# MurpheyLab/trep

Measured on AMD Instinct MI355X. Metric: DEL-steps/sec x batch (puppet ~40-DOF, fp64), higher is better.
Workload: dtype f64

## Files before the change

trep_amd/csrc/mvi_core.hpp:

```cpp
#pragma once
#include <cmath>

#include "program.hpp"
#include "dual.hpp"
#include "lanes.hpp"

#if defined(TG_MOCK_TIMING) || defined(TG_MOCK_REAL_LDS) || defined(TG_MOCK_LDS_D1) || defined(TG_MOCK_LDS_D2) || \
    defined(TG_BBD_FUSED_UPDATE) || defined(TG_BBD_INLINE) || defined(TG_BBD_ASM) || \
    defined(TG_WEV_NO_RC_IDENT) || defined(TG_WEV_CLEAR_EARLY) || defined(TG_WEV_MERGE_C) || \
    defined(TG_NO_BBD) || defined(TG_NO_CMP) || defined(TG_NO_GJ_PANEL) || defined(TG_NO_QUAD_SWEEP) || defined(TG_NO_DUAL_SWEEP) || \
    defined(TG_NO_AB_MFMA) || defined(TG_NO_HZ_MFMA) || defined(GJR_EXEC32) || defined(GJP_SKIP_STEPS) || defined(GJP_SKIP_UPDATE) || \
    defined(TG_FRESH_PHASES) || defined(TG_FRESH_STEP) || \
    defined(TG_CHAIN_PRIO) || defined(TG_PREFIX_GROUP) || defined(TG_LT_TRIPS) || defined(TG_ROLLOUT_WAVES) || defined(TG_DERIV_WAVES)
#error "a retired experiment switch is defined (TG_MOCK_*, TG_BBD_FUSED_UPDATE / _INLINE / _ASM, TG_WEV_*, TG_NO_* except TG_NO_WEV, GJR_ / GJP_*, TG_FRESH_*, or a former -D tunable): these variants were removed -- verdicts in docs/LOG.md, their source in commit 89f6ce0"
#endif

#if defined(TG_HELPER_WAVES)
constexpr int TG_NW = TG_HELPER_WAVES;
#else
constexpr int TG_NW = 1;
#endif

#if defined(__HIPCC__)
__device__ __forceinline__ double *tg_lds_base() {
// ... 48 lines not shown
template <class P> struct tg_is_spec<P, typename std::enable_if<(P::nq >= 0)>::type> { static constexpr bool value = true; };
template <class P, class = void> struct tg_items_aligned { static constexpr bool value = false; };
template <class P> struct tg_items_aligned<P, typename std::enable_if<(P::nq >= 0)>::type> { static constexpr bool value = (P::o_J % 2 == 0) && (P::o_W % 2 == 0); };
template <class P, class = void> struct tg_static_sweep { static constexpr bool value = false; };
template <class P> struct tg_static_sweep<P, typename std::enable_if<(P::sw_ok > 0)>::type> { static constexpr bool value = true; };
template <class P, class = void> struct tg_static_cmp { static constexpr bool value = false; };
template <class P> struct tg_static_cmp<P, typename std::enable_if<(P::cmp_ok >= 0)>::type> { static constexpr bool value = P::cmp_ok != 0 && P::tab_ok != 0; };

template <class P, class = void> struct tg_static_wev { static constexpr bool value = false; };
#if !defined(TG_NO_WEV)
template <class P> struct tg_static_wev<P, typename std::enable_if<(P::wev_ok >= 0)>::type> { static constexpr bool value = P::wev_ok != 0 && P::cmp_ok != 0 && P::tab_ok != 0; };
#endif

template <class P, class = void> struct tg_static_pk { static constexpr bool value = false; };
#if defined(TG_BBD_PACKED)
template <class P> struct tg_static_pk<P, typename std::enable_if<(P::bbd_pk_ok >= 0)>::type> { static constexpr bool value = P::bbd_pk_ok != 0 && tg_static_wev<P>::value && tg_static_bbd<P>::value; };
#endif

template <class P, class = void> struct tg_static_fb { static constexpr bool value = false; };
template <class P> struct tg_static_fb<P, typename std::enable_if<(P::fb_on >= 0)>::type> { static constexpr bool value = P::fb_on != 0 && tg_static_wev<P>::value; };

template <class P, class = void> struct tg_static_tr { static constexpr bool value = false; };
template <class P> struct tg_static_tr<P, typename std::enable_if<(P::tr_on >= 0)>::type> { static constexpr bool value = P::tr_on != 0 && tg_static_sweep<P>::value && P::tab_ok != 0; };

enum { MODE_ROLLOUT = 0, MODE_CALC_P2 = 1, MODE_CALC_F = 2, MODE_DERIV1 = 3, MODE_DERIV2Z = 4, MODE_DYNAMICS = 5, MODE_DYN_DERIV1 = 6, MODE_ENERGY = 7, MODE_LAGRANGIAN = 8 };

struct RunArgs {
    int batch, n_steps, max_iterations, mode;
    int predictor;
    double dt, t1, t2, tolerance;
    double *q1, *q2, *p1, *p2, *lam, *u1;
    const double *U, *K;
    const double *q2_hint, *lam_hint;
    const double *Kproj, *bX, *bU;
    double *Uout;
    int group_size;
    const int *group_map;
    double *X;
    double *f_out;
    double *d1[12];
    double *A_out, *B_out;
    const double *z;
    double *hz;
    int *iters, *status;
    long long *prof_out;
    const double *dt_steps;
// ... 352 lines not shown
                TG_SYNC();
            }
            return;
        }
#endif
        for (int L = 1; L < P.n_levels; L++) {
            const int l0 = P.level_off[L], cnt = P.level_off[L + 1] - l0;
            if (on) TG_FOR(idx, 4 * cnt) {
                const int j = P.lvl_joints[l0 + (idx >> 2)], cc = idx & 3;
                if (P.j_parent[j] < 0) continue;
                const Real *gp = G + 12 * P.j_parent[j];
                Real *gj = G + 12 * j;
                const Real m0 = gj[cc], m1 = gj[4 + cc], m2 = gj[8 + cc], u3 = (cc == 3) ? 1.0 : 0.0;
                const Real v0 = gp[0] * m0 + gp[1] * m1 + gp[2] * m2 + u3 * gp[3];
                const Real v1 = gp[4] * m0 + gp[5] * m1 + gp[6] * m2 + u3 * gp[7];
                const Real v2 = gp[8] * m0 + gp[9] * m1 + gp[10] * m2 + u3 * gp[11];
                gj[cc] = v0; gj[4 + cc] = v1; gj[8 + cc] = v2;
            }
            TG_SYNC();
        }
    }

#if defined(__HIP_DEVICE_COMPILE__)
    TG_HD void pose_sweep_dual(bool on, bool rollout_lists) {
        const int sjn = rollout_lists ? P.n_sj : 2 * P.n_joints;
        double *sc = S + P.o_sc, *sc2 = S + P.o_J, *G = S + P.o_G, *G2 = S + P.o_W;
        const int nj = P.n_joints;
        const int n12 = 12 * nj, n24 = 2 * n12;
        SwDesc sw0;
        if constexpr (tg_static_sweep<typename std::remove_cv<PROG>::type>::value) {
            if (rollout_lists) sw0 = sw_fetch<typename std::remove_cv<PROG>::type, 0>((const int *)(S + SwPlan<typename std::remove_cv<PROG>::type>::o_sched()));
        }
        constexpr bool TR = tg_static_tr<typename std::remove_cv<PROG>::type>::value;
        if (P.tab_ok) {
            double pr[2][12];
            int trw[2] = {0, 0};
#pragma unroll
            for (int u = 0; u < 2; u++) {
                const double *src = (TR && rollout_lists ? P.tr_prm : P.j_prm) + 12 * (size_t)((jck[u] >> 16) & 0xFFF);
#pragma unroll
                for (int e = 0; e < 12; e++) pr[u][e] = src[e];
                if constexpr (TR) { if (rollout_lists) trw[u] = P.tr_sj[lane + u * TEAM < sjn ? lane + u * TEAM : 0]; }
            }
            if (on) {
#pragma unroll
                for (int u = 0; u < 2; u++) {
                    const int idx = lane + u * TEAM;
                    if (u * TEAM < sjn && idx < sjn) {
                        const bool second = (jck[u] >> 28) != 0;
                        const int j = (jck[u] >> 16) & 0xFFF, kind = (jck[u] >> 12) & 0xF;
                        const double x = qval(second ? dsB : dsA, jck[u] & 0xFFF);
                        const bool rotary = kind >= TG_RX;
                        const int a = rotary ? kind - TG_RX : kind - TG_TX, b = a == 2 ? 0 : a + 1, c = a == 0 ? 2 : a - 1;
                        double *g = (second ? G2 : G) + 12 * j;
                        auto row_t = [&](int l, double v) {
                            if constexpr (TR) {
                                typedef typename std::remove_cv<PROG>::type SP;
                                constexpr int ROWS = tg_static_wev<SP>::value ? SP::tr_rows : 7;
                                if (rollout_lists && ((ROWS >> l) & 1)) { const double e = qval(second ? dsB : dsA, (trw[u] >> (8 * l)) & 0xFF); return (trw[u] >> (24 + l)) & 1 ? e : v; }
                            }
                            return v;
                        };
                        if (u * TEAM < sc_rot2) {
                            double sn = 0.0, cs = 1.0;
                            if (rotary) tg_sincos(x, &sn, &cs);
                            const double tq = rotary ? 0.0 : x;
#pragma unroll
                            for (int l = 0; l < 3; l++) {
                                const double A_ = pr[u][4 * l], B_ = pr[u][4 * l + 1], C_ = pr[u][4 * l + 2], D_ = pr[u][4 * l + 3];
                                g[4 * l + a] = A_;
                                g[4 * l + b] = rotary ? fma(C_, sn, B_ * cs) : B_;
// ... 520 lines not shown
        v += tg_dpp_f64<0x111>(v); v += tg_dpp_f64<0x112>(v); v += tg_dpp_f64<0x114>(v); v += tg_dpp_f64<0x118>(v);
        double norm2 = tg_readlane_f64(v, 15);
        if (P.nd > 16) norm2 += tg_readlane_f64(v, 31);
        if (P.nd > 32) norm2 += tg_readlane_f64(v, 47);
        if (P.nd > 48) norm2 += tg_readlane_f64(v, 63);
        return !(norm2 > tolerance * tolerance) && !__any(res_hoff ? 1 : 0);
    }

    template <int D0, int D1> TG_HD void wev_sum(const double *SU, double (&V)[6]) const {
        if constexpr (D0 < D1) {
            double x[D1 - D0][6];
#pragma unroll
            for (int d = D0; d < D1; d++) {
                const int idx = (wvl[d >> 2] >> (8 * (d & 3))) & 0xFF;
                ld6<true>(SU + 6 * idx, x[d - D0]);
            }
#pragma unroll
            for (int d = D0; d < D1; d++) {
#pragma unroll
                for (int r = 0; r < 6; r++) V[r] += x[d - D0][r];
            }
        }
    }
    TG_HD void eval_world(bool on) {
        typedef typename std::remove_cv<PROG>::type SP;
        constexpr bool FB = tg_static_fb<SP>::value;
        constexpr int nd = SP::nd, NB = SP::n_bodies, NG = SP::n_cgroups, MAXD = FB ? SP::fb_depth : SP::wev_depth;
        static_assert(TEAM == 64 && nd + 3 * NB < 64, "eval_world: one lane per config and per (body, axis), and the last lane free");
        static_assert(!FB || nd + 3 * NB < 63, "eval_world: the prefix record needs a second lane without a role");
        constexpr int NREC = (SP::o_ccz - SP::o_csw) / 12;
        static_assert((SP::o_ccz - SP::o_csw) % 12 == 0 && NREC == nd + (FB ? 2 : 1), "eval_world: the twist area holds nd + 1 records, nd + 2 with a prefix");
        static_assert((SP::o_csw & 1) == 0 && ((SP::o_csw + 6 * NREC) & 1) == 0 && (SP::o_I & 1) == 0 && (SP::o_cmp & 1) == 0 && (SP::o_G & 1) == 0, "eval_world: 16-byte LDS accesses");
        const int l0 = tg_opaque(lane);
        const bool blane = l0 >= nd && l0 < nd + 3 * NB;
        const int wb_ = blane ? wvl[3] & 0xFF : 0, wr_ = blane ? (wvl[3] >> 8) & 3 : 0;
        double eo0, eo1, eo2, eor; int eanc;
        {
            const int ii = l0 < 3 * P.n_endpoints ? l0 : 0;
            const double *o = P.ae_d + 4 * (size_t)ii;
            eo0 = o[0]; eo1 = o[1]; eo2 = o[2]; eor = o[3]; eanc = P.ae_i[ii];
        }
        double Cb[12];
#pragma unroll
        for (int e = 0; e < 12; e++) Cb[e] = P.b_C[12 * (size_t)wb_ + e];
        const int banc = P.b_anchor[wb_];
        if (!rates_ready) {
            if (on) TG_FOR(i, P.nq) S[P.o_dq + i] = (S[P.o_q2 + i] - S[P.o_q1 + i]) / dt;
            TG_RSYNC();
        }
        TG_STAMP(0);
        pose_sweep_dual(on, true);
        TG_STAMP(1);
        const double *G = S + P.o_G, *G2 = S + P.o_W;
        double *SW = S + P.o_csw, *SU = SW + 6 * NREC, *CMP = S + P.o_cmp, *BW = S + P.o_W + 12 * P.n_joints;
        constexpr int BWS = 17;
        static_assert(12 * SP::n_joints + BWS * NB <= 6 * SP::n_items + 9 * NB, "eval_world: body entries do not fit behind the q2 poses");
        const ConTab ct = fetch_constraints();
        double bD0 = 0.0, bD1 = 0.0, bD2 = 0.0, bC0 = 0.0, bC1 = 0.0, bC2 = 0.0, bm = 0.0;
        if (on) {
            if (lane < 3 * P.n_endpoints) {
                const int r = lane % 3;
                const double *g = G2 + 12 * (eanc < 0 ? 0 : eanc) + 4 * r;
                const double val = g[0] * eo0 + g[1] * eo1 + g[2] * eo2 + g[3];
                S[P.o_pE + lane] = eanc < 0 ? eor : val;
            }
            if (lane < nd || lane == TEAM - 1 || (FB && lane == TEAM - 2)) {
                const bool real = lane < nd;
                const int rec = real ? lane : (FB && lane == TEAM - 2 ? nd + 1 : nd);
                const int oj = real ? wvl[3] & 0xFFFF : 0, kind = real ? (wvl[3] >> 16) & 0xFF : (int)TG_TX;
                const bool prismatic = kind <= TG_TZ;
                const int ax = prismatic ? kind - TG_TX : kind - TG_RX;
                const double *gj = G + oj;
                const double a0 = gj[ax], a1 = gj[4 + ax], a2 = gj[8 + ax];
                const double px = gj[3], py = gj[7], pz = gj[11];
// ... 2760 lines not shown
        if (live && lane == 0) { A.iters[t] = 0; A.status[t] = ok ? TG_OK : TG_SINGULAR; }
    }
    if constexpr (MODE == MODE_DYNAMICS) {
        const bool ok = core.dynamics(live, A, t);
        if (live && lane == 0) { A.iters[t] = 0; A.status[t] = ok ? TG_OK : TG_SINGULAR; }
    }
}

template <int TEAM, int MODE, bool SPRINGS = false, class PROG = CProg, class ARGS = CArgs, int PIVOT = -1, bool PAR = false>
TG_HD void run_trajectory(PROG &P0, ARGS &A0, double *S, int lane, int traj, int wave = 0, int nw = 1, const ParTable T = ParTable{nullptr, 1, 0}) {
    PROG &P = P0;
    ARGS &A = A0;
    const int nq = P.nq, nd = P.nd, nk = P.nk, nu = P.nu, nc = P.nc;
    const bool live = traj < A.batch;
    const size_t t = (size_t)(live ? traj : 0);
    double dt = MODE == MODE_ROLLOUT ? A.dt : (A.t2 - A.t1);
    if (A.dt_steps && A.dt_period > 0) dt = A.dt_steps[t % (size_t)A.dt_period];
    Core<TEAM, SPRINGS, PROG, double, PAR> core(P, S, lane, dt);
    if constexpr (PAR) core.par = T.rows + (t / (size_t)T.group) * (size_t)T.stride + 4 * P.n_bodies;
    else (void)T;
    core.wave = wave; core.nw = nw;
    core.d1_compact = MODE == MODE_DERIV1 && P.a_ok != 0;
    if (wave == 0) core.init_sweep_schedule(MODE == MODE_ROLLOUT);
#if defined(TG_PROFILE) && defined(__HIP_DEVICE_COMPILE__)
    core.prof_last = (long long)__builtin_amdgcn_s_memtime();
    const long long prof_rt0 = (long long)__builtin_amdgcn_s_memrealtime();
#endif

    if (live && wave == 0) {
        TG_FOR(i, nq) { S[P.o_q1 + i] = A.q1[t * nq + i]; S[P.o_q2 + i] = A.q2[t * nq + i]; }
        TG_FOR(i, nd) S[P.o_p1 + i] = (MODE == MODE_ROLLOUT) ? A.p2[t * nd + i] : A.p1[t * nd + i];
        TG_FOR(i, nc) S[P.o_lam + i] = A.lam[t * nc + i];
        TG_FOR(i, nu) S[P.o_u + i] = A.u1[t * nu + i];
        TG_FOR(i, P.n_dh) { S[P.o_Dh1 + i] = 0.0; S[P.o_Dh2 + i] = 0.0; }
    }
    TG_SYNC();

    if constexpr (MODE == MODE_CALC_P2) {
        core.eval_midpoint(live);
        if (live) TG_FOR(i, nd) A.p2[t * nd + i] = 0.5 * dt * S[P.o_Ldq + i] + S[P.o_Lddq + i];
        return;
    }
    if constexpr (MODE == MODE_DERIV1) {
        core.deriv1(live, A, t);
        return;
    }
// ... 158 lines not shown
        if (!edged) {
        if (fuse_rates && on) TG_FOR(i, nq) S[P.o_dq + i] = core.over_dt(S[P.o_q2 + i] - S[P.o_q1 + i]);
        if (step == 0) core.eval_constraints(on, 1, false, S + P.o_Dh1);
        else if (nc) {
            if (on) TG_FOR(i, P.n_dh) S[P.o_Dh1 + i] = S[P.o_Dh2 + i];
            TG_RSYNC();
        }
        }
        int iterations = 0;
        bool done = !on;
        pre_ok = false;
        if (TEAM == 64 && on && !A.Kproj && nu <= TEAM && nk <= TEAM && step + 1 < A.n_steps) {
            if (lane < nu) pre_u = A.U[(t * A.n_steps + step + 1) * nu + lane];
            if (pre_kl >= 0 && pre_kl < nk) pre_k = A.K[(t * A.n_steps + step + 1) * nk + pre_kl];
            pre_ok = true;
        }
#if defined(TG_PROFILE) && defined(__HIP_DEVICE_COMPILE__)
        { long long t_ = (long long)__builtin_amdgcn_s_memtime(); core.prof[9] += t_ - core.prof_last; core.prof_last = t_; }
#endif
        for (;;) {
            PROG &P = tg_rebind(P0);
            const int nd = P.nd, nc = P.nc;
#if defined(__HIP_DEVICE_COMPILE__)
            if constexpr (TEAM == 64 && !SPRINGS && tg_static_wev<typename std::remove_cv<PROG>::type>::value) { core.wev_on = true; core.pk_image = PIVOT == 0; core.eval_world(!done); }
            else if (core.dual_ok()) { if (P.tab_ok) core.eval_both_tab(!done); else core.eval_both(!done); }
            else
#endif
            {
                core.eval_midpoint(!done);
                core.eval_constraints(!done, 2, true, S + P.o_Dh2);
            }
#if defined(__HIP_DEVICE_COMPILE__)
            if (core.dual_ok() && P.tab_ok) { if (!done && core.solved_fused(A.tolerance)) done = true; }
            else
#endif
            if (!done && core.solved(A.tolerance)) done = true;
#if defined(TG_PROFILE) && defined(__HIP_DEVICE_COMPILE__)
            { long long t_ = (long long)__builtin_amdgcn_s_memtime(); core.prof[12] += t_ - core.prof_last; core.prof_last = t_; }
#endif
            if (!done && iterations > A.max_iterations) { done = true; failed = true; status = TG_NOT_CONVERGED; }
#if defined(__HIP_DEVICE_COMPILE__)
            if (TEAM == 64 ? done : (__all(done ? 1 : 0) != 0)) break;
#else
            if (done) break;
#endif
#if defined(__HIP_DEVICE_COMPILE__)
            BbdRows<tg_static_bbd_cols<TEAM == 64 && PIVOT == 0, typename std::remove_cv<PROG>::type>::value> bbd_tab_rows;
// ... 172 lines not shown
```

trep_amd/csrc/program.hpp:

```cpp
#pragma once
#include "../../include/trep_amd.h"

namespace tg {

struct DevProg {
#define TG_F_INT(name) int name;
#define TG_F_ARRAY(type, name, n) type name[n];
#define TG_F_TABLE(type, name) const type *name;
#include "devprog_fields.def"
#undef TG_F_INT
#undef TG_F_ARRAY
#undef TG_F_TABLE
};

constexpr int kCmpRecord = 16, kCmpStride = 18;
static_assert(kCmpStride >= kCmpRecord && kCmpStride % 2 == 0 && kCmpRecord % 2 == 0, "composite records: 16-byte aligned");
template <class SP> constexpr int cmp_stride() {
    static_assert(SP::n_cgroups > 0 && (SP::o_csw - SP::o_cmp) % SP::n_cgroups == 0, "composite records: o_csw is not a whole number of strides behind o_cmp");
    constexpr int stride = (SP::o_csw - SP::o_cmp) / SP::n_cgroups;
    static_assert((stride == kCmpRecord || stride == kCmpStride) && (SP::o_cmp & 1) == 0, "composite records: stride");
    return stride;
}

}

#ifndef __HIPCC__
#include "schedule.hpp"
#endif
```

trep_amd/csrc/schedule.hpp:

```cpp
#pragma once
#include <algorithm>
#include <cmath>
#include <cstdio>
#include <cstdlib>
#include <cstring>
#include <functional>
#include <map>
#include <stdexcept>
#include <string>
#include <vector>

#include "program.hpp"
#include "bbd.hpp"

namespace tg {

struct HostProgram {
    DevProg p{};
#define TG_F_INT(name)
#define TG_F_ARRAY(type, name, n)
#define TG_F_TABLE(type, name) std::vector<type> name;
#include "devprog_fields.def"
#undef TG_F_INT
#undef TG_F_ARRAY
#undef TG_F_TABLE
    std::vector<unsigned char> newton_pattern;
    int max_depth = 0;
    std::vector<int> frame_anchor;
    std::vector<double> frame_offset;
    std::vector<int> ipool;
    std::vector<double> dpool;
    std::vector<size_t> toff;
    void pack();
    void bind(DevProg &P, const int *I, const double *D) const;
};

namespace detail {
struct M34 {
    double m[12];
};
inline M34 ident() {
    M34 r{};
    r.m[0] = r.m[5] = r.m[10] = 1.0;
    return r;
}
inline M34 mul(const M34 &a, const M34 &b) {
    M34 r{};
    for (int i = 0; i < 3; i++)
        for (int j = 0; j < 4; j++) {
            double s = (j == 3) ? a.m[4 * i + 3] : 0.0;
            for (int k = 0; k < 3; k++) s += a.m[4 * i + k] * b.m[4 * k + j];
            r.m[4 * i + j] = s;
// ... 28 lines not shown
    DevProg &P;
    const int nfr, nq, nd, nc;
    int n_levels = 0, nj = 0, nb = 0, nitems = 0;
    int n_true_springs = 0, ns = 0, nw = 0, nel = 0;
    int n_dh_con = 0, n_dh_spr = 0, n_cpair_con = 0, n_cpair_spr = 0;
    bool has_plane = false;
    std::vector<int> jorder, joint_of_frame, joint_of_cfg;
    std::vector<int> anchor;
    std::vector<M34> offset;
    std::map<int, int> ep_of_frame;
    int cmp_stride = kCmpRecord;
    std::vector<int> pose_need;
    int off = 0;
    static constexpr int kCompositeMinNd = 8;
    int take(int n) { int o = off; off += (n > 0 ? n : 0); return o; }

    explicit ScheduleBuilder(const tg_system_desc *desc) : d(desc), P(H.p), nfr(desc->n_frames), nq(desc->n_configs), nd(desc->n_dyn), nc(desc->n_constraints) {}
    int endpoint(int f);
    void check_desc(), number_joints(), joint_tables(), bodies_and_items();
    void constraints(), springs_and_point_forces(), element_tables(), forces_and_potentials();
    void counts_and_step_layout(), sweep_lists_and_plan(), layout_pose_union_and_deriv1();
    void body_chunks(), helper_wave_lists(), layout_derivatives();
    void composite_form(), floating_base_tables(const std::vector<std::vector<int>> &lists), world_eval();
    void structured_solve(), translation_runs();
};

inline int ScheduleBuilder::endpoint(int f) {
    auto it = ep_of_frame.find(f);
    if (it != ep_of_frame.end()) return it->second;
    int e = (int)H.e_anchor.size();
    ep_of_frame[f] = e;
    H.e_anchor.push_back(anchor[f]);
    H.e_off.push_back(offset[f].m[3]); H.e_off.push_back(offset[f].m[7]); H.e_off.push_back(offset[f].m[11]);
    return e;
}

inline void ScheduleBuilder::check_desc() {
    if (nd + d->n_kin != nq) throw std::runtime_error("n_dyn + n_kin != n_configs");
    for (int f = 0; f < nfr; f++) {
        int t = d->frame_transform[f];
        if (t < TG_WORLD || t > TG_CONST_SE3) throw std::runtime_error("unknown frame transform");
        if (d->frame_config[f] >= 0 && (t < TG_TX || t > TG_RZ)) throw std::runtime_error("config on a non-parametric frame");
        if (f > 0 && (d->frame_parent[f] < 0 || d->frame_parent[f] >= f)) throw std::runtime_error("frames must be listed parent-first");
    }
}

inline void ScheduleBuilder::number_joints() {
// ... 806 lines not shown
            const int first = H.ch_first[c] + k, len = H.ch_len[c] - k, parent = k ? first - 1 : H.ch_parent[c];
            if (len == 0) continue;
            w[0] = (12 * first) | (len << 16); w[1] = parent >= 0 ? 12 * parent : -1;
            for (int set = 0; set < 2; set++) if (pose_need[first] >> set & 1) inst.push_back(slot | (set << 8) | (1 << 9));
        }
        P.tr_np[r] = ((int)inst.size() + 4) / 5;
        for (int p = 0; p < P.tr_np[r]; p++) {
            int len = 0;
            for (int q = 0; q < 5 && 5 * p + q < (int)inst.size(); q++) {
                P.tr_inst[(4 * r + p) * 5 + q] = inst[5 * p + q];
                len = std::max(len, H.tr_sched[2 * (size_t)(16 * r + (inst[5 * p + q] & 0xFF))] >> 16);
            }
            P.tr_len[4 * r + p] = len;
            P.tr_maxlen = std::max(P.tr_maxlen, len);
        }
    }
    if (on) {
        P.tr_on = 1;
        P.o_sched2 = P.lds_per_team;
        P.lds_per_team += 16 * P.n_rounds;
    }
    if (H.tr_joint.empty()) { H.tr_joint.push_back(0); H.tr_src.assign(3, -1); H.tr_const.assign(3, 0.0); }
}
}

inline HostProgram build_program(const tg_system_desc *d) {
    detail::ScheduleBuilder b(d);
    b.check_desc(); b.number_joints(); b.joint_tables(); b.bodies_and_items();
    b.constraints(); b.springs_and_point_forces(); b.element_tables(); b.forces_and_potentials();
    b.counts_and_step_layout(); b.sweep_lists_and_plan(); b.layout_pose_union_and_deriv1();
    b.body_chunks(); b.helper_wave_lists(); b.layout_derivatives();
    b.composite_form(); b.world_eval(); b.structured_solve(); b.translation_runs();
    b.H.pack();
    return std::move(b.H);
}

namespace detail {
template <typename T>
inline size_t pool_append(std::vector<T> &pool, const std::vector<T> &v) {
    const size_t at = pool.size();
    pool.insert(pool.end(), v.begin(), v.end());
    while (pool.size() % 4) pool.push_back(T());
    return at;
}
inline std::vector<int> &pool_of(std::vector<int> &I, std::vector<double> &, int) { return I; }
inline std::vector<double> &pool_of(std::vector<int> &, std::vector<double> &D, double) { return D; }
inline const int *pool_of(const int *I, const double *, int) { return I; }
inline const double *pool_of(const int *, const double *D, double) { return D; }
inline std::string spec_value(int v) { return std::to_string(v); }
inline std::string spec_value(double v) { char t[40]; std::snprintf(t, sizeof(t), "%a", v); return t; }
template <typename T>
inline void emit_spec_pool(std::string &out, const char *decl, const std::vector<T> &pool, size_t per_line) {
    out += decl + std::to_string(pool.size()) + "] = {";
    for (size_t i = 0; i < pool.size(); i++) out += (i ? ((i % per_line) ? "," : ",\n") : "\n") + spec_value(pool[i]);
    out += "};\n";
// ... 44 lines not shown
    DevProg P = H.p;
    H.bind(P, H.ipool.data(), H.dpool.data());
    out += "// specialised schedule: sizes, counts, LDS offsets and tables as compile-time constants\n";
    detail::emit_spec_pool(out, "__device__ const int spec_ipool[", H.ipool, 32);
    detail::emit_spec_pool(out, "__device__ const double spec_dpool[", H.dpool, 8);
    out += "struct SpecProg {\n";
#define TG_F_INT(name) out += "    static constexpr int " #name " = " + std::to_string(P.name) + ";\n";
#define TG_F_ARRAY(type, name, n)
#define TG_F_TABLE(type, name)
#include "devprog_fields.def"
#undef TG_F_INT
#undef TG_F_ARRAY
#define TG_F_INT(name)
#define TG_F_ARRAY(type, name, n) detail::emit_spec_array(out, #type, #name, P.name, n);
#include "devprog_fields.def"
#undef TG_F_ARRAY
#undef TG_F_TABLE
#define TG_F_ARRAY(type, name, n)
#define TG_F_TABLE(type, name) detail::emit_spec_pointer(out, #type, #name, P.name, H);
#include "devprog_fields.def"
#undef TG_F_INT
#undef TG_F_ARRAY
#undef TG_F_TABLE
    out += "};\n";
}

}
```

trep_amd/csrc/spec_kernel.hip:

```cpp
#include <hip/hip_runtime.h>

#include <type_traits>

#define TG_GJ_PANEL_DEFAULT 1
#include "mvi_core.hpp"
#include TG_SPEC_HEADER

namespace {
#if defined(SPEC_ARGS_IN_MEMORY)
#define SPEC_KERNEL_ARGS const tg::RunArgs *__restrict__ Ag
#define SPEC_ARGS_REF tg::KArgs &A = *(tg::KArgs *)Ag
#else
#define SPEC_KERNEL_ARGS const tg::RunArgs A
#define SPEC_ARGS_REF ((void)0)
#endif

template <int MODE> constexpr int spec_waves() { return ((MODE == tg::MODE_DERIV1 || MODE == tg::MODE_DERIV2Z) && SPEC_TEAM == 64) ? TG_NW : 1; }
static_assert(TG_NW >= 1 && TG_NW <= 2, "helper waves: the pair lists of program.hpp are split in exactly two parts (wave_part, wp_* / wt_* / wcp4)");
static_assert(TG_NW == 1 || SPEC_TEAM == 64, "helper waves are for full-wave teams (trep_amd/specialize.py passes TG_HELPER_WAVES only then)");

constexpr int TG_ROLLOUT_WAVES = 2;
constexpr int TG_DERIV_WAVES = 1;
template <int MODE, int PIVOT = 0>
__global__ __launch_bounds__(64 * spec_waves<MODE>(), MODE == tg::MODE_DERIV1 ? (SpecProg::a_ok ? 2 : 1) : (MODE == tg::MODE_DERIV2Z ? TG_DERIV_WAVES : TG_ROLLOUT_WAVES)) void k_spec(SPEC_KERNEL_ARGS) {
// ... 95 lines not shown
#else
    hipLaunchKernelGGL((k_spec_par<MODE, PIVOT>), dim3(grid), dim3(64 * spec_waves<MODE>()), lds, stream, *A, T);
#endif
    return hipGetLastError() == hipSuccess ? 0 : 1;
}
}

extern "C" {
const int *tg_spec_sizes(void) {
    static const int s[8] = {(int)sizeof(tg::DevProg), (int)sizeof(tg::RunArgs), SpecProg::nq, SpecProg::nd, SpecProg::nc, SpecProg::n_items,
                             SpecProg::n_pairs, SpecProg::lds_per_team};
    return s;
}
unsigned long long tg_spec_key(void) {
#if defined(TG_SPEC_KEY)
    return TG_SPEC_KEY;
#else
    return 0ull;
#endif
}
int tg_spec_waves(void) { return spec_waves<tg::MODE_DERIV2Z>(); }
int tg_spec_fb_n(void) { return tg::tg_static_fb<SpecProg>::value ? SpecProg::fb_n : 0; }
int tg_spec_tr_n(void) { return tg::tg_static_tr<SpecProg>::value ? SpecProg::tr_n : 0; }
int tg_spec_modes(void) {
    int m = 1 << tg::MODE_ROLLOUT;
#if defined(SPEC_DERIVATIVES)
    m |= (1 << tg::MODE_DERIV1) | (1 << tg::MODE_DERIV2Z);
#endif
    return m;
}
int tg_spec_par_modes(void) { return tg_spec_modes(); }
int tg_spec_debug_solve(const double *A_dev, double *x_dev, int *path_dev, int n_mats, int skip_structured) {
    const size_t lds = sizeof(double) * (size_t)SpecProg::lds_per_team;
    if (lds > 64 * 1024 &&
        hipFuncSetAttribute(reinterpret_cast<const void *>(&k_spec_debug_solve), hipFuncAttributeMaxDynamicSharedMemorySize, (int)lds) != hipSuccess) return 1;
    hipLaunchKernelGGL(k_spec_debug_solve, dim3(n_mats), dim3(64), lds, 0, A_dev, x_dev, path_dev, skip_structured);
    return hipGetLastError() == hipSuccess ? 0 : 1;
}
int tg_spec_launch(int mode, const tg::RunArgs *A, tg::RunArgs *device_slot, int grid, size_t lds, void *stream) {
    switch (mode) {
    case tg::MODE_ROLLOUT:
        return A->exact_pivot ? launch_mode<tg::MODE_ROLLOUT, 1>(A, device_slot, grid, lds, (hipStream_t)stream)
                              : launch_mode<tg::MODE_ROLLOUT, 0>(A, device_slot, grid, lds, (hipStream_t)stream);
#if defined(SPEC_DERIVATIVES)
    case tg::MODE_DERIV1: return launch_mode<tg::MODE_DERIV1>(A, device_slot, grid, lds, (hipStream_t)stream);
    case tg::MODE_DERIV2Z: return launch_mode<tg::MODE_DERIV2Z>(A, device_slot, grid, lds, (hipStream_t)stream);
// ... 19 lines not shown
```

trep_amd/csrc/trepamd.hip:

```cpp
#include <hip/hip_runtime.h>

#include <cmath>
#include <cstdio>
#include <cstdlib>
#include <cstring>
#include <memory>
#include <string>
#include <vector>

#include "device_buffer.hpp"
#include "launch_generic.hpp"
#include "mvi_project.hpp"
#include "mvi_equilibrium.hpp"
#include "mvi_inverse.hpp"
#include "mvi_frames.hpp"
#include "mvi_tape.hpp"
#include "mvi_dyn_inverse.hpp"
#include "schedule.hpp"
#include <dlfcn.h>

namespace tg_detail {
int launch_par(int team, bool springs, const tg::DevProg *d_prog, const tg::RunArgs &A, const tg::ParTable &T, int grid, size_t lds, hipStream_t stream);
int launch_project(int team, bool springs, const tg::DevProg *d_prog, const tg::RunArgs &A, const tg::ProjectArgs &J, int grid, size_t lds, hipStream_t stream);
int launch_equilibrium(int team, bool springs, bool par, const tg::DevProg *d_prog, const tg::RunArgs &A, const tg::EquilibriumArgs &J, const tg::ParTable &T, int grid, size_t lds, hipStream_t stream);
// ... 50 lines not shown

struct tg_batch {
    tg_system *sys = nullptr;
    int batch = 0, device = 0;
    tg::DevProg P{};
    tg::DeviceBuffer<tg::DevProg> d_prog;
    void *spec_lib = nullptr;
    int (*spec_launch)(int, const tg::RunArgs *, tg::RunArgs *, int, size_t, void *) = nullptr;
    int (*spec_launch_par)(int, const tg::RunArgs *, tg::RunArgs *, int, size_t, void *, const double *, int, int) = nullptr;
    int spec_par_modes = 0;
    tg::DeviceBuffer<double> par_dev;
    int par_rows = 0, par_group = 1, par_stride = 0;
    struct Launched { unsigned int modes = 0; long long n = 0; void add(int mode) { modes |= 1u << mode; n++; } } launched[2][2];
    static constexpr int ARG_SLOTS = 4;
    tg::DeviceBuffer<tg::RunArgs> d_args;
    tg::PinnedBuffer<tg::RunArgs> h_args;
    tg::Event arg_done[ARG_SLOTS];
    bool arg_used[ARG_SLOTS] = {false, false, false, false};
    int arg_next = 0;
    tg::PinnedBuffer<double> io_host;
    double *io_dev = nullptr;
    size_t io_in = 0, io_out = 0;
    bool mirror_valid = false;
    int spec_modes = 0, spec_waves = 1, spec_fb_n = 0, spec_tr_n = 0;
    std::string spec_path;
    tg::DeviceBuffer<int> d_ints;
    tg::DeviceBuffer<double> d_dbls;
    tg::DeviceBuffer<double> q1, q2, p1, p2, lam, u1;
    tg::DeviceBuffer<double> stage_u, stage_k, stage_qh, stage_lh, f_out;
    tg::DeviceBuffer<int> iters, status, fallbacks;
    tg::DeviceBuffer<double> z_dev, hz_dev, zl_dev;
    tg::DeviceBuffer<double> dyn;
    tg::DeviceBuffer<double> dyn_d1;
    tg::DeviceBuffer<double> energy;
    tg::DeviceBuffer<double> lag;
    tg::DeviceBuffer<int> dyn_ints;
    tg::DeviceBuffer<double> pose;
    tg::DeviceBuffer<int> pose_ints;
    std::vector<int32_t> frames_sel;
    std::vector<int> frames_tab_host;
    std::vector<double> frames_off_host;
    tg::DeviceBuffer<int> frames_tab;
    tg::DeviceBuffer<double> frames_off;
    std::vector<int32_t> tape_start, tape_sel;
    tg::TapeTable tape_host;
    tg::DeviceBuffer<int> tape_words;
    tg::DeviceBuffer<double> tape_off;
// ... 1815 lines not shown
    const tg::DevProg &P = b->P;
    const int want[8] = {(int)sizeof(tg::DevProg), (int)sizeof(tg::RunArgs), P.nq, P.nd, P.nc, P.n_items, P.n_pairs, P.lds_per_team};
    const int *got = sizes_fn();
    for (int i = 0; i < 8; i++) if (got[i] != want[i]) return fail(TG_ERR_INVALID, "specialised kernel was built for a different system or library version");
    if (key_fn() != tg_system_spec_key(b->sys)) return fail(TG_ERR_INVALID, "specialised kernel was built from a different schedule (header hash mismatch)");
    if (!b->d_args) {
        tg::DeviceBuffer<tg::RunArgs> d_args;
        tg::PinnedBuffer<tg::RunArgs> h_args;
        tg::Event done[tg_batch::ARG_SLOTS];
        bool ok = d_args.ensure(tg_batch::ARG_SLOTS) == hipSuccess && h_args.ensure(tg_batch::ARG_SLOTS, hipHostMallocDefault) == hipSuccess;
        for (int i = 0; i < tg_batch::ARG_SLOTS && ok; i++) ok = done[i].create(hipEventDisableTiming) == hipSuccess;
        if (!ok) return fail(TG_ERR_HIP, "allocation of the argument blocks failed");
        b->d_args = std::move(d_args); b->h_args = std::move(h_args);
        for (int i = 0; i < tg_batch::ARG_SLOTS; i++) b->arg_done[i] = std::move(done[i]);
    }
    if (b->spec_lib) { hipStreamSynchronize(b->stream); dlclose(b->spec_lib); }
    b->spec_lib = lib.release(); b->spec_launch = launch_fn; b->spec_modes = modes_fn(); b->spec_path = library_path;
    auto waves_fn = reinterpret_cast<int (*)(void)>(dlsym(h, "tg_spec_waves"));
    b->spec_waves = waves_fn ? waves_fn() : 1;
    auto fb_fn = reinterpret_cast<int (*)(void)>(dlsym(h, "tg_spec_fb_n"));
    b->spec_fb_n = fb_fn ? fb_fn() : 0;
    auto tr_fn = reinterpret_cast<int (*)(void)>(dlsym(h, "tg_spec_tr_n"));
    b->spec_tr_n = tr_fn ? tr_fn() : 0;
    auto par_fn = reinterpret_cast<int (*)(int, const tg::RunArgs *, tg::RunArgs *, int, size_t, void *, const double *, int, int)>(dlsym(h, "tg_spec_launch_par"));
    auto par_modes_fn = reinterpret_cast<int (*)(void)>(dlsym(h, "tg_spec_par_modes"));
    b->spec_launch_par = par_modes_fn ? par_fn : nullptr;
    b->spec_par_modes = (par_fn && par_modes_fn) ? par_modes_fn() : 0;
    return TG_SUCCESS;
}

int tg_system_newton_plan(const tg_system *sys, int32_t out[8], uint8_t *pattern, int32_t *tab) {
    if (!sys || !out) return fail(TG_ERR_INVALID, "null argument");
    const tg::DevProg &P = sys->H.p;
    out[0] = P.bbd_ok; out[1] = P.bbd_g; out[2] = P.bbd_ng; out[3] = P.bbd_nb; out[4] = P.bbd_t; out[5] = P.nf; out[6] = P.nd; out[7] = 0;
    if (pattern) {
        std::memset(pattern, 0, (size_t)P.nf * P.nf);
        if (sys->H.newton_pattern.size() == (size_t)P.nf * P.nf) std::memcpy(pattern, sys->H.newton_pattern.data(), sys->H.newton_pattern.size());
    }
    if (tab) for (int i = 0; i < 128; i++) tab[i] = i < (int)sys->H.bbd_tab.size() ? sys->H.bbd_tab[i] : 0;
    return TG_SUCCESS;
}

int tg_batch_debug_newton_solve(tg_batch *b, int32_t n_mats, int32_t skip_structured, const double *A_aug_host, double *x_host, int32_t *path_host) {
    if (!b || n_mats <= 0 || !A_aug_host || !x_host || !path_host) return fail(TG_ERR_INVALID, "bad arguments");
    if (!b->spec_lib) return fail(TG_ERR_INVALID, "no specialised kernel library loaded");
    auto fn = reinterpret_cast<int (*)(const double *, double *, int *, int, int)>(dlsym(b->spec_lib, "tg_spec_debug_solve"));
    if (!fn) return fail(TG_ERR_INVALID, "the specialised library has no solve hook");
    const int nf = b->P.nf;
    HIP_TRY(hipSetDevice(b->device));
    tg::DeviceBuffer<double> dA, dx;
    tg::DeviceBuffer<int> dp;
    const size_t cA = (size_t)n_mats * nf * (nf + 1), cx = (size_t)n_mats * nf, cp = (size_t)n_mats;
    auto failed = [](const char *what) { (void)hipGetLastError(); return fail(TG_ERR_HIP, what); };
    if (dA.ensure(cA) != hipSuccess || dx.ensure(cx) != hipSuccess || dp.ensure(cp) != hipSuccess) return failed("solve hook: device allocation failed");
    if (hipMemcpy(dA.get(), A_aug_host, cA * sizeof(double), hipMemcpyHostToDevice) != hipSuccess) return failed("solve hook: upload failed");
    const int rc = fn(dA.get(), dx.get(), dp.get(), n_mats, skip_structured);
    if (hipDeviceSynchronize() != hipSuccess || rc != 0) return failed("solve hook launch failed");
    if (hipMemcpy(x_host, dx.get(), cx * sizeof(double), hipMemcpyDeviceToHost) != hipSuccess ||
        hipMemcpy(path_host, dp.get(), cp * sizeof(int), hipMemcpyDeviceToHost) != hipSuccess)
        return failed("solve hook: download failed");
    return TG_SUCCESS;
}

int tg_batch_info(const tg_batch *b, int32_t out[8]) {
    if (!b || !out) return fail(TG_ERR_INVALID, "null argument");
    out[0] = b->spec_launch ? b->spec_modes : 0;
    for (int spec = 0; spec < 2; spec++) { out[2 - spec] = (int32_t)b->launched[0][spec].modes; out[4 - spec] = (int32_t)std::min<long long>(b->launched[0][spec].n, 0x7fffffff); }
    out[5] = b->exact_pivot; out[6] = b->sys->team; out[7] = b->spec_launch ? b->spec_waves : 1;
    if (b->spec_launch) out[7] |= (b->spec_fb_n << 8) | ((b->spec_tr_n & 0xFF) << 16);
    return TG_SUCCESS;
}

int tg_batch_par_info(const tg_batch *b, int32_t out[8]) {
    if (!b || !out) return fail(TG_ERR_INVALID, "null argument");
    out[0] = b->spec_launch_par ? b->spec_par_modes : 0;
    for (int spec = 0; spec < 2; spec++) { out[2 - spec] = (int32_t)b->launched[1][spec].modes; out[4 - spec] = (int32_t)std::min<long long>(b->launched[1][spec].n, 0x7fffffff); }
    out[5] = b->par_rows; out[6] = b->par_rows ? b->par_group : 0; out[7] = 0;
    return TG_SUCCESS;
}

int tg_system_parameters(const tg_system *sys, int32_t sizes_out[4], double *inertia, double *gravity, double *damping) {
    if (!sys) return fail(TG_ERR_INVALID, "null system");
    const tg::HostProgram &H = sys->H;
    if (sizes_out) { sizes_out[0] = H.p.n_bodies; sizes_out[1] = H.p.nd; sizes_out[2] = sys->has_gravity; sizes_out[3] = sys->has_damping; }
    const int nb = H.p.n_bodies, nd = H.p.nd;
    std::vector<double> row(4 * (size_t)nb + 3 + nd);
    base_parameter_row(H, row.data());
    if (inertia) std::copy_n(row.begin(), 4 * nb, inertia);
    if (gravity) std::copy_n(row.begin() + 4 * nb, 3, gravity);
    if (damping) std::copy_n(row.begin() + 4 * nb + 3, nd, damping);
    return TG_SUCCESS;
}
// ... 64 lines not shown
```

trep_amd/midpointvi.py:

```python
import collections
import os

import numpy as np

from . import _lib
from .descriptor import flatten
from .errors import ConvergenceError

Projection = collections.namedtuple("Projection", "Q dQ mu iterations status")
Equilibrium = collections.namedtuple("Equilibrium", "Q mu V iterations status")
InverseDynamics = collections.namedtuple("InverseDynamics", "U lam P rho h status")
FrameKinematics = collections.namedtuple("FrameKinematics", "g vb p_dq vb_ddq")
TapeMeasures = collections.namedtuple("TapeMeasures", "length velocity length_dq velocity_dq length_dqdq")
DynamicsInverse = collections.namedtuple("DynamicsInverse", "U lam rho tau acc status")
InverseDynamicsRank = collections.namedtuple("InverseDynamicsRank", "U lam P rho h status rank")
DynamicsInverseRank = collections.namedtuple("DynamicsInverseRank", "U lam rho tau acc status rank")
InverseDynamicsBounded = collections.namedtuple("InverseDynamicsBounded", "U lam P rho h status rank active solves")
DynamicsInverseBounded = collections.namedtuple("DynamicsInverseBounded", "U lam rho tau acc status rank active solves")


class BatchMidpointVI(object):

    def __init__(self, system, batch, tolerance=1e-10, device=0, specialize="auto"):
        self._system = system
# ... 114 lines not shown
        _lib.check(self._L.tg_batch_set_pivot_rule(self._h, 1 if value else 0))
        self._exact_pivot = bool(value)

    system = property(lambda self: self._system)
    batch = property(lambda self: self._batch)
    device = property(lambda self: self._device)
    nq = property(lambda self: int(self._desc.n_configs))
    nd = property(lambda self: int(self._desc.n_dyn))
    nk = property(lambda self: int(self._desc.n_kin))
    nu = property(lambda self: int(self._desc.n_inputs))
    nc = property(lambda self: int(self._desc.n_constraints))
    nX = property(lambda self: self.nq + self.nd + self.nk)
    nU = property(lambda self: self.nu + self.nk)

    def info(self):
        out = (np.zeros(8, dtype=np.int32))
        _lib.check(self._L.tg_system_info(self._sys_h, out.ctypes.data_as(_lib._c_ip)))
        keys = ["team", "lds_bytes_per_trajectory", "joints", "levels", "bodies", "items", "pairs", "dh_items"]
        d = dict(zip(keys, (int(v) for v in out)))
        kout = np.zeros(8, dtype=np.int32)
        _lib.check(self._L.tg_batch_info(self._h, kout.ctypes.data_as(_lib._c_ip)))
        d["fb_n"] = (int(kout[7]) >> 8) & 0xFF
        d["tr_n"] = (int(kout[7]) >> 16) & 0xFF
        return d

    MODES = {"rollout": 0, "calc_p2": 1, "calc_f": 2, "deriv1": 3, "deriv2z": 4}
    ALL_MODES = dict(MODES, dynamics=5, dynamics_deriv1=6, energy=7, lagrangian=8)

    def parameters(self):
        sizes = np.zeros(4, dtype=np.int32)
        _lib.check(self._L.tg_system_parameters(self._sys_h, sizes.ctypes.data, None, None, None))
        inertia = np.zeros((int(sizes[0]), 4))
        gravity, damping = np.zeros(3), np.zeros(int(sizes[1]))
        _lib.check(self._L.tg_system_parameters(self._sys_h, None, inertia.ctypes.data if inertia.size else None, gravity.ctypes.data,
                                                damping.ctypes.data if damping.size else None))
        return {"inertia": inertia, "gravity": gravity if sizes[2] else None, "damping": damping if sizes[3] else None}

    def set_parameters(self, inertia=None, gravity=None, damping=None, group=1):
        self.refresh()
        from . import parameters as _par
        rows, group, blocks = _par.pack(self._system, self._batch, inertia=inertia, gravity=gravity, damping=damping, group=group)
        p = lambda name: None if blocks[name] is None or blocks[name].size == 0 else blocks[name].ctypes.data
        rc = self._L.tg_batch_set_parameters(self._h, rows, group, p("inertia"), p("gravity"), p("damping"))
        if rc == _lib.ERR_INVALID:
            raise ValueError(self._L.tg_last_error().decode())
        _lib.check(rc)
        self._parameter_rows = rows

    def clear_parameters(self):
        _lib.check(self._L.tg_batch_clear_parameters(self._h))
        self._parameter_rows = 0

    @property
    def has_parameters(self):
        return getattr(self, "_parameter_rows", 0) > 0

    def kernel_info(self):
        out = np.zeros(8, dtype=np.int32)
        _lib.check(self._L.tg_batch_info(self._h, out.ctypes.data_as(_lib._c_ip)))
        names = lambda bits: sorted(n for n, m in self.MODES.items() if (int(bits) >> m) & 1)
        par = np.zeros(8, dtype=np.int32)
        _lib.check(self._L.tg_batch_par_info(self._h, par.ctypes.data_as(_lib._c_ip)))
        every = lambda bits: sorted(n for n, m in self.ALL_MODES.items() if (int(bits) >> m) & 1)
        return {"spec_modes": names(out[0]), "spec_launched": names(out[1]), "generic_launched": names(out[2]),
                "spec_launch_mask": int(out[1]), "generic_launch_mask": int(out[2]),
                "spec_launches": int(out[3]), "generic_launches": int(out[4]), "exact_pivot": bool(out[5]), "team": int(out[6]),
                "helper_waves": int(out[7]) & 0xFF, "fb_n": (int(out[7]) >> 8) & 0xFF, "tr_n": (int(out[7]) >> 16) & 0xFF, "spec_library": self._specialized,
                "par_spec_modes": every(par[0]), "par_spec_launched": every(par[1]), "par_generic_launched": every(par[2]),
                "par_spec_launch_mask": int(par[1]), "par_generic_launch_mask": int(par[2]), "par_spec_launches": int(par[3]), "par_generic_launches": int(par[4]), "parameter_rows": int(par[5]),
                "parameter_group": int(par[6])}

    @property
    def stream(self):
        return self._L.tg_batch_stream(self._h)

    @property
    def tolerance(self):
        return self._tolerance

    @tolerance.setter
    def tolerance(self, value):
        self._tolerance = float(value)
        _lib.check(self._L.tg_batch_set_tolerance(self._h, self._tolerance))

    def times(self):
        import ctypes
        a, b = ctypes.c_double(), ctypes.c_double()
        _lib.check(self._L.tg_batch_get_times(self._h, ctypes.byref(a), ctypes.byref(b)))
        return a.value, b.value

# ... 853 lines not shown
```

Before: 60.70 million.

## Carry unchanged joint poses into the first Newton iterate instead of resweeping

Adds a host-side analysis that finds joints whose pose depends only on kinematic/fixed coordinates or on translation runs. For the first Newton iteration of a rollout step it replaces the full dual pose sweep with a cheap pass: it rebuilds only the translation-dependent poses and copies the rest from the q2 pose area into the q1 area. It also extends the ordinary sweep with extra lanes, so poses without a q2 twin are still produced. This aims to cut redundant trig and chain composition per step, at the cost of more spec-time logic and a narrower set of qualifying systems.

```diff
diff --git a/trep_amd/csrc/mvi_core.hpp b/trep_amd/csrc/mvi_core.hpp
--- a/trep_amd/csrc/mvi_core.hpp
+++ b/trep_amd/csrc/mvi_core.hpp
@@ -94,6 +94,9 @@
 
 template <class P, class = void> struct tg_static_tr { static constexpr bool value = false; };
 template <class P> struct tg_static_tr<P, typename std::enable_if<(P::tr_on >= 0)>::type> { static constexpr bool value = P::tr_on != 0 && tg_static_sweep<P>::value && P::tab_ok != 0; };
+
+template <class P, class = void> struct tg_static_carry { static constexpr bool value = false; static constexpr int n = 0; };
+template <class P> struct tg_static_carry<P, typename std::enable_if<(P::pc_on >= 0)>::type> { static constexpr bool value = P::pc_on != 0 && tg_static_tr<P>::value && tg_static_wev<P>::value; static constexpr int n = value ? P::pc_n : 0; };
 
 enum { MODE_ROLLOUT = 0, MODE_CALC_P2 = 1, MODE_CALC_F = 2, MODE_DERIV1 = 3, MODE_DERIV2Z = 4, MODE_DYNAMICS = 5, MODE_DYN_DERIV1 = 6, MODE_ENERGY = 7, MODE_LAGRANGIAN = 8 };
 
@@ -492,7 +495,7 @@
     }
 
 #if defined(__HIP_DEVICE_COMPILE__)
-    TG_HD void pose_sweep_dual(bool on, bool rollout_lists) {
+    template <bool CARRYL = false> TG_HD void pose_sweep_dual(bool on, bool rollout_lists) {
         const int sjn = rollout_lists ? P.n_sj : 2 * P.n_joints;
         double *sc = S + P.o_sc, *sc2 = S + P.o_J, *G = S + P.o_G, *G2 = S + P.o_W;
         const int nj = P.n_joints;
@@ -511,12 +514,13 @@
 #pragma unroll
                 for (int e = 0; e < 12; e++) pr[u][e] = src[e];
                 if constexpr (TR) { if (rollout_lists) trw[u] = P.tr_sj[lane + u * TEAM < sjn ? lane + u * TEAM : 0]; }
+                if constexpr (CARRYL) { if (lane + u * TEAM >= sjn) trw[u] = 0; }
             }
             if (on) {
 #pragma unroll
                 for (int u = 0; u < 2; u++) {
                     const int idx = lane + u * TEAM;
-                    if (u * TEAM < sjn && idx < sjn) {
+                    if (u * TEAM < sjn && idx < (CARRYL ? sjn + tg_static_carry<typename std::remove_cv<PROG>::type>::n : sjn)) {
                         const bool second = (jck[u] >> 28) != 0;
                         const int j = (jck[u] >> 16) & 0xFFF, kind = (jck[u] >> 12) & 0xF;
                         const double x = qval(second ? dsB : dsA, jck[u] & 0xFFF);
@@ -1083,7 +1087,50 @@
             }
         }
     }
-    TG_HD void eval_world(bool on) {
+    TG_HD void pose_carry_pass(bool on) {
+        typedef typename std::remove_cv<PROG>::type SP;
+        static_assert((SP::o_G & 1) == 0 && (SP::o_W & 1) == 0, "carried poses: the 16-byte copy G2 -> G needs both pose areas on an even double");
+        double *G = S + P.o_G, *G2 = S + P.o_W;
+        const int l = tg_opaque(lane);
+        if (on && l < SP::n_sj) {
+            const int w = jck[0];
+            const bool second = (w >> 28) != 0;
+            const int j = (w >> 16) & 0xFFF;
+            if (((l < 32 ? SP::pc_kin_0 : SP::pc_kin_1) >> (l & 31)) & 1) {
+                const int a = ((w >> 12) & 0xF) - TG_TX, b = a == 2 ? 0 : a + 1, c = a == 0 ? 2 : a - 1;
+                const double x = qval(second ? dsB : dsA, w & 0xFFF);
+                const double *src = P.tr_prm + 12 * (size_t)j;
+                const int tw = P.tr_sj[l];
+                double *g = (second ? G2 : G) + 12 * j;
+#pragma unroll
+                for (int r = 0; r < 3; r++) {
+                    const double A_ = src[4 * r], B_ = src[4 * r + 1], C_ = src[4 * r + 2], D_ = src[4 * r + 3];
+                    double t = fma(A_, x, D_);
+                    if ((SP::tr_rows >> r) & 1) { const double e = qval(second ? dsB : dsA, (tw >> (8 * r)) & 0xFF); t = (tw >> (24 + r)) & 1 ? e : t; }
+                    g[4 * r + a] = A_; g[4 * r + b] = B_; g[4 * r + c] = C_; g[4 * r + 3] = t;
+                }
+            } else if (!second) {
+                typedef double tg_d2 __attribute__((ext_vector_type(2)));
+                const tg_d2 *from = reinterpret_cast<const tg_d2 *>(G2 + 12 * j);
+                tg_d2 *to = reinterpret_cast<tg_d2 *>(G + 12 * j);
+                tg_d2 v[6];
+#pragma unroll
+                for (int e = 0; e < 6; e++) v[e] = from[e];
+#pragma unroll
+                for (int e = 0; e < 6; e++) to[e] = v[e];
+            }
+        }
+        TG_RSYNC();
+        TG_STAMP(5);
+        TG_STAMP(15);
+    }
+    TG_HD void init_carry_lanes() {
+        typedef typename std::remove_cv<PROG>::type SP;
+        static_assert(TEAM == 64 && SP::n_sj + SP::pc_n <= TEAM && SP::pc_n <= kPoseCarryMax, "carried poses: the items without a q2 twin fit the first trip");
+        const int l = tg_opaque(lane);
+        if (l >= SP::n_sj && l < SP::n_sj + SP::pc_n) jck[0] = SP::pc_item[l - SP::n_sj];
+    }
+    TG_HD void eval_world(bool on, bool carry = false) {
         typedef typename std::remove_cv<PROG>::type SP;
         constexpr bool FB = tg_static_fb<SP>::value;
         constexpr int nd = SP::nd, NB = SP::n_bodies, NG = SP::n_cgroups, MAXD = FB ? SP::fb_depth : SP::wev_depth;
@@ -1110,7 +1157,8 @@
             TG_RSYNC();
         }
         TG_STAMP(0);
-        pose_sweep_dual(on, true);
+        if constexpr (tg_static_carry<SP>::value) { if (carry) pose_carry_pass(on); else pose_sweep_dual<true>(on, true); }
+        else pose_sweep_dual(on, true);
         TG_STAMP(1);
         const double *G = S + P.o_G, *G2 = S + P.o_W;
         double *SW = S + P.o_csw, *SU = SW + 6 * NREC, *CMP = S + P.o_cmp, *BW = S + P.o_W + 12 * P.n_joints;
@@ -3917,6 +3965,9 @@
     core.wave = wave; core.nw = nw;
     core.d1_compact = MODE == MODE_DERIV1 && P.a_ok != 0;
     if (wave == 0) core.init_sweep_schedule(MODE == MODE_ROLLOUT);
+#if defined(__HIP_DEVICE_COMPILE__)
+    if constexpr (MODE == MODE_ROLLOUT && TEAM == 64 && !SPRINGS && tg_static_carry<typename std::remove_cv<PROG>::type>::value) core.init_carry_lanes();
+#endif
 #if defined(TG_PROFILE) && defined(__HIP_DEVICE_COMPILE__)
     core.prof_last = (long long)__builtin_amdgcn_s_memtime();
     const long long prof_rt0 = (long long)__builtin_amdgcn_s_memrealtime();
@@ -4121,7 +4172,11 @@
             PROG &P = tg_rebind(P0);
             const int nd = P.nd, nc = P.nc;
 #if defined(__HIP_DEVICE_COMPILE__)
-            if constexpr (TEAM == 64 && !SPRINGS && tg_static_wev<typename std::remove_cv<PROG>::type>::value) { core.wev_on = true; core.pk_image = PIVOT == 0; core.eval_world(!done); }
+            if constexpr (TEAM == 64 && !SPRINGS && tg_static_wev<typename std::remove_cv<PROG>::type>::value) {
+                core.wev_on = true; core.pk_image = PIVOT == 0;
+                if constexpr (tg_static_carry<typename std::remove_cv<PROG>::type>::value) core.eval_world(!done, edged && iterations == 0);
+                else core.eval_world(!done);
+            }
             else if (core.dual_ok()) { if (P.tab_ok) core.eval_both_tab(!done); else core.eval_both(!done); }
             else
 #endif
diff --git a/trep_amd/csrc/program.hpp b/trep_amd/csrc/program.hpp
--- a/trep_amd/csrc/program.hpp
+++ b/trep_amd/csrc/program.hpp
@@ -22,6 +22,13 @@
     return stride;
 }
 
+constexpr int kPoseCarryMax = 8;
+struct PoseCarry {
+    int on = 0, n = 0;
+    int item[kPoseCarryMax] = {0, 0, 0, 0, 0, 0, 0, 0};
+    unsigned kin[2] = {0u, 0u};
+};
+
 }
 
 #ifndef __HIPCC__
diff --git a/trep_amd/csrc/schedule.hpp b/trep_amd/csrc/schedule.hpp
--- a/trep_amd/csrc/schedule.hpp
+++ b/trep_amd/csrc/schedule.hpp
@@ -28,6 +28,7 @@
     int max_depth = 0;
     std::vector<int> frame_anchor;
     std::vector<double> frame_offset;
+    PoseCarry carry;
     std::vector<int> ipool;
     std::vector<double> dpool;
     std::vector<size_t> toff;
@@ -102,7 +103,7 @@
     void counts_and_step_layout(), sweep_lists_and_plan(), layout_pose_union_and_deriv1();
     void body_chunks(), helper_wave_lists(), layout_derivatives();
     void composite_form(), floating_base_tables(const std::vector<std::vector<int>> &lists), world_eval();
-    void structured_solve(), translation_runs();
+    void structured_solve(), translation_runs(), pose_carry();
 };
 
 inline int ScheduleBuilder::endpoint(int f) {
@@ -955,6 +956,40 @@
     }
     if (H.tr_joint.empty()) { H.tr_joint.push_back(0); H.tr_src.assign(3, -1); H.tr_const.assign(3, 0.0); }
 }
+inline void ScheduleBuilder::pose_carry() {
+    PoseCarry &C = H.carry;
+    C = PoseCarry();
+    if (!P.tr_on || P.n_sj > 64) return;
+    std::vector<int> run(nj, 0), moved(nj, 0);
+    for (int i = 0; i < P.tr_n; i++) run[H.tr_joint[i]] = 1;
+    for (int j = 0; j < nj; j++) moved[j] = (H.j_cfg[j] >= nd ? 1 : 0) | (H.j_parent[j] >= 0 ? moved[H.j_parent[j]] : 0);
+    for (int n = 0; n < P.n_sj; n++) {
+        const int j = (H.sj_list[n] >> 16) & 0xFFF;
+        if (!moved[j]) continue;
+        if (!run[j]) { C = PoseCarry(); return; }
+        C.kin[n >> 5] |= 1u << (n & 31);
+    }
+    int n = 0, item[kPoseCarryMax];
+    for (int k = 0; k < nj; k++) {
+        if ((pose_need[k] & 3) != 1) continue;
+        if (n == kPoseCarryMax || moved[k] || run[k]) { C = PoseCarry(); return; }
+        bool swept = false;
+        for (int r = 0; r < P.n_rounds && !swept; r++)
+            for (int c = H.round_off[r]; c < H.round_off[r + 1] && !swept; c++) {
+                if (k < H.ch_first[c] || k >= H.ch_first[c] + H.ch_len[c]) continue;
+                const int slot = c - H.round_off[r];
+                if (slot >= 16) break;
+                const int w = H.tr_sched[2 * (size_t)(16 * r + slot)], first = (w & 0xFFFF) / 12, len = w >> 16;
+                if (k < first || k >= first + len) break;
+                for (int i = 0; i < 20; i++) if (P.tr_inst[20 * r + i] == (slot | (1 << 8) | (1 << 9))) swept = true;
+            }
+        if (!swept) { C = PoseCarry(); return; }
+        item[n++] = H.j_cfg[k] | (H.j_kind[k] << 12) | (k << 16) | (1 << 28);
+    }
+    if (P.n_sj + n > 64) { C = PoseCarry(); return; }
+    C.on = 1; C.n = n;
+    for (int i = 0; i < n; i++) C.item[i] = item[i];
+}
 }
 
 inline HostProgram build_program(const tg_system_desc *d) {
@@ -963,7 +998,7 @@
     b.constraints(); b.springs_and_point_forces(); b.element_tables(); b.forces_and_potentials();
     b.counts_and_step_layout(); b.sweep_lists_and_plan(); b.layout_pose_union_and_deriv1();
     b.body_chunks(); b.helper_wave_lists(); b.layout_derivatives();
-    b.composite_form(); b.world_eval(); b.structured_solve(); b.translation_runs();
+    b.composite_form(); b.world_eval(); b.structured_solve(); b.translation_runs(); b.pose_carry();
     b.H.pack();
     return std::move(b.H);
 }
@@ -1054,6 +1089,12 @@
 #undef TG_F_INT
 #undef TG_F_ARRAY
 #undef TG_F_TABLE
+    if (H.carry.on) {
+        const PoseCarry &C = H.carry;
+        out += "    static constexpr int pc_on = 1;\n    static constexpr int pc_n = " + std::to_string(C.n) + ";\n";
+        out += "    static constexpr int pc_kin_0 = " + std::to_string((int)C.kin[0]) + ";\n    static constexpr int pc_kin_1 = " + std::to_string((int)C.kin[1]) + ";\n";
+        detail::emit_spec_array(out, "int", "pc_item", C.item, kPoseCarryMax);
+    }
     out += "};\n";
 }
 
diff --git a/trep_amd/csrc/spec_kernel.hip b/trep_amd/csrc/spec_kernel.hip
--- a/trep_amd/csrc/spec_kernel.hip
+++ b/trep_amd/csrc/spec_kernel.hip
@@ -141,6 +141,7 @@
 int tg_spec_waves(void) { return spec_waves<tg::MODE_DERIV2Z>(); }
 int tg_spec_fb_n(void) { return tg::tg_static_fb<SpecProg>::value ? SpecProg::fb_n : 0; }
 int tg_spec_tr_n(void) { return tg::tg_static_tr<SpecProg>::value ? SpecProg::tr_n : 0; }
+int tg_spec_pose_carry(void) { return tg::tg_static_carry<SpecProg>::value ? 1 | (tg::tg_static_carry<SpecProg>::n << 1) : 0; }
 int tg_spec_modes(void) {
     int m = 1 << tg::MODE_ROLLOUT;
 #if defined(SPEC_DERIVATIVES)
diff --git a/trep_amd/csrc/trepamd.hip b/trep_amd/csrc/trepamd.hip
--- a/trep_amd/csrc/trepamd.hip
+++ b/trep_amd/csrc/trepamd.hip
@@ -96,7 +96,7 @@
     double *io_dev = nullptr;
     size_t io_in = 0, io_out = 0;
     bool mirror_valid = false;
-    int spec_modes = 0, spec_waves = 1, spec_fb_n = 0, spec_tr_n = 0;
+    int spec_modes = 0, spec_waves = 1, spec_fb_n = 0, spec_tr_n = 0, spec_pose_carry = 0;
     std::string spec_path;
     tg::DeviceBuffer<int> d_ints;
     tg::DeviceBuffer<double> d_dbls;
@@ -1958,6 +1958,8 @@
     b->spec_fb_n = fb_fn ? fb_fn() : 0;
     auto tr_fn = reinterpret_cast<int (*)(void)>(dlsym(h, "tg_spec_tr_n"));
     b->spec_tr_n = tr_fn ? tr_fn() : 0;
+    auto pc_fn = reinterpret_cast<int (*)(void)>(dlsym(h, "tg_spec_pose_carry"));
+    b->spec_pose_carry = pc_fn ? pc_fn() : 0;
     auto par_fn = reinterpret_cast<int (*)(int, const tg::RunArgs *, tg::RunArgs *, int, size_t, void *, const double *, int, int)>(dlsym(h, "tg_spec_launch_par"));
     auto par_modes_fn = reinterpret_cast<int (*)(void)>(dlsym(h, "tg_spec_par_modes"));
     b->spec_launch_par = par_modes_fn ? par_fn : nullptr;
@@ -2003,7 +2005,7 @@
     out[0] = b->spec_launch ? b->spec_modes : 0;
     for (int spec = 0; spec < 2; spec++) { out[2 - spec] = (int32_t)b->launched[0][spec].modes; out[4 - spec] = (int32_t)std::min<long long>(b->launched[0][spec].n, 0x7fffffff); }
     out[5] = b->exact_pivot; out[6] = b->sys->team; out[7] = b->spec_launch ? b->spec_waves : 1;
-    if (b->spec_launch) out[7] |= (b->spec_fb_n << 8) | ((b->spec_tr_n & 0xFF) << 16);
+    if (b->spec_launch) out[7] |= (b->spec_fb_n << 8) | ((b->spec_tr_n & 0xFF) << 16) | ((b->spec_pose_carry & 0x1F) << 24);
     return TG_SUCCESS;
 }
 
diff --git a/trep_amd/midpointvi.py b/trep_amd/midpointvi.py
--- a/trep_amd/midpointvi.py
+++ b/trep_amd/midpointvi.py
@@ -160,6 +160,8 @@
         _lib.check(self._L.tg_batch_info(self._h, kout.ctypes.data_as(_lib._c_ip)))
         d["fb_n"] = (int(kout[7]) >> 8) & 0xFF
         d["tr_n"] = (int(kout[7]) >> 16) & 0xFF
+        d["pose_carry"] = bool((int(kout[7]) >> 24) & 1)
+        d["n_carry"] = (int(kout[7]) >> 25) & 0xF
         return d
 
     MODES = {"rollout": 0, "calc_p2": 1, "calc_f": 2, "deriv1": 3, "deriv2z": 4}
@@ -203,7 +205,8 @@
         return {"spec_modes": names(out[0]), "spec_launched": names(out[1]), "generic_launched": names(out[2]),
                 "spec_launch_mask": int(out[1]), "generic_launch_mask": int(out[2]),
                 "spec_launches": int(out[3]), "generic_launches": int(out[4]), "exact_pivot": bool(out[5]), "team": int(out[6]),
-                "helper_waves": int(out[7]) & 0xFF, "fb_n": (int(out[7]) >> 8) & 0xFF, "tr_n": (int(out[7]) >> 16) & 0xFF, "spec_library": self._specialized,
+                "helper_waves": int(out[7]) & 0xFF, "fb_n": (int(out[7]) >> 8) & 0xFF, "tr_n": (int(out[7]) >> 16) & 0xFF,
+                "pose_carry": bool((int(out[7]) >> 24) & 1), "n_carry": (int(out[7]) >> 25) & 0xF, "spec_library": self._specialized,
                 "par_spec_modes": every(par[0]), "par_spec_launched": every(par[1]), "par_generic_launched": every(par[2]),
                 "par_spec_launch_mask": int(par[1]), "par_generic_launch_mask": int(par[2]), "par_spec_launches": int(par[3]), "par_generic_launches": int(par[4]), "parameter_rows": int(par[5]),
                 "parameter_group": int(par[6])}
```

Result: faster. 61.55 million, median of 6 (+1.4%).
